# rapidsai/cugraph

Measured on NVIDIA H100. Metric: MTEPS (million traversed edges/sec) PageRank RMAT-24 ef-16, 100 iterations, higher is better.
Workload: dtype f32

## Files before the change

cugraph_b200/csrc/graph.cuh:

```cuda
#pragma once
#include "common.cuh"

#include <memory>
#include <vector>

namespace b200 {

constexpr int kNumSeg                = 7;
constexpr int kSegThreshold[kNumSeg] = {32, 16, 8, 4, 2, 1, 0};

constexpr int kWarpChunk  = 1024;
constexpr int kWarpsPerCta = 8;

struct sweep_cache_t;

struct csx_t {
  int32_t n_rows{0};
  int64_t nnz{0};
  bool offs64{false};
  dbuf offsets;
  dbuf indices;
  dbuf weights;
  dbuf row_vertex;
  bool degree_sorted{true};
  int32_t seg[kNumSeg + 1]{};
  int64_t nnz_hi{0};
  int32_t n_chunks{0};
  dbuf chunk_first_row;
  int32_t n_split{0};
  dbuf split_rows;
  mutable std::unique_ptr<sweep_cache_t> sweep;
  mutable dbuf out_w;
  csx_t();
  ~csx_t();
};

struct graph_impl {
  cugraph_data_type_id_t vertex_type{INT32};
  cugraph_data_type_id_t edge_type{INT32};
  cugraph_data_type_id_t weight_type{FLOAT32};
  bool weighted{false};
  bool is_symmetric{false};
  bool is_multigraph{false};
  bool store_transposed{false};
  bool renumbered{true};
  int32_t n_vertices{0};
  int64_t n_edges{0};
  int device{0};

  dbuf ext_of_int;
  dbuf sorted_ext;
  dbuf int_of_rank;

  std::unique_ptr<csx_t> primary;
  std::unique_ptr<csx_t> pull_alt;
  std::unique_ptr<csx_t> push_alt;
  std::unique_ptr<csx_t> out_alt;
};

inline graph_impl* G(cugraph_graph_t* g)
{
  B200_EXPECTS(g != nullptr, CUGRAPH_INVALID_INPUT, "graph is NULL");
  return reinterpret_cast<graph_impl*>(g);
}

csx_t const& pull_view(handle_impl const& h, graph_impl& g);
csx_t const& push_view(handle_impl const& h, graph_impl& g);
csx_t const& out_sweep_view(handle_impl const& h, graph_impl& g);

struct pr_state_t {
  double diff;
  double dangling;
  double init;
  double pers_scale;
  double last_diff;
  int iter;
  int done;
};
struct sweep_scratch_t {
  dbuf acc, state;
  void init(handle_impl const& h, csx_t const& c);
  void set_init(handle_impl const& h, double init);
  pr_state_t* st() const { return state.as<pr_state_t>(); }
};
size_t padded_x_elems(int32_t n_vertices, size_t elem_size);
template <typename T>
dbuf make_sweep_x(handle_impl const& h, int32_t n_vertices);
template <typename T>
void pull_sweep(handle_impl const& h, csx_t const& c, int32_t n_vertices, T const* x, T* y, sweep_scratch_t& sc, double alpha,
                bool use_weights = true, bool covered_rows_only = false);
void prepare_pull_sweep(handle_impl const& h, csx_t const& c, int32_t n_vertices, size_t elem_size);

void ext_to_int(handle_impl const& h, graph_impl const& g, void const* ext, size_t n, int32_t* out);
void int_to_ext(handle_impl const& h, graph_impl const& g, int32_t const* in, size_t n, void* ext_out);
dbuf reported_vertices(handle_impl const& h, graph_impl const& g);
dbuf to_reported_order(handle_impl const& h, graph_impl const& g, void const* internal_vals, size_t elem_size);

template <typename T>
dbuf collect_vertex_values(handle_impl const& h, graph_impl const& g,
                           device_array_view_impl const* verts, device_array_view_impl const* vals,
                           T fill);

std::unique_ptr<csx_t> build_binned_rows(handle_impl const& h, int32_t const* major, int32_t const* minor, void const* w,
                                         cugraph_data_type_id_t wtype, int64_t n, int32_t nv);
dbuf expand_majors(handle_impl const& h, csx_t const& c);

}
```

cugraph_b200/csrc/pagerank.cu:

```cuda
#include "graph.cuh"

#include <algorithm>
#include <cmath>

namespace b200 {
namespace {

__global__ void k_out_degree(int32_t const* __restrict__ indices, long long nnz, int32_t* __restrict__ deg)
{
  for (long long i = blockIdx.x * (long long)blockDim.x + threadIdx.x; i < nnz; i += (long long)gridDim.x * blockDim.x)
    atomicAdd(deg + indices[i], 1);
}

template <typename T>
__global__ void k_out_weight(int32_t const* __restrict__ indices, T const* __restrict__ w, long long nnz, double* __restrict__ sums)
{
  for (long long i = blockIdx.x * (long long)blockDim.x + threadIdx.x; i < nnz; i += (long long)gridDim.x * blockDim.x)
    atomicAdd(sums + indices[i], (double)w[i]);
}

template <typename S, typename T>
__global__ void k_cast(S const* in, int32_t n, T* out)
{
  for (int64_t i = blockIdx.x * (int64_t)blockDim.x + threadIdx.x; i < n; i += (int64_t)gridDim.x * blockDim.x) out[i] = (T)in[i];
// ... 1 lines not shown

template <typename T>
__global__ void __launch_bounds__(kBlock)
k_vertex_pass(T const* __restrict__ pr_new, T const* __restrict__ pr_old, T const* __restrict__ out_w,
              T* __restrict__ x, int32_t n, pr_state_t* __restrict__ st)
{
  if (st->done) return;
  __shared__ double smem[8];
  double diff = 0.0, dang = 0.0;
  for (int i = blockIdx.x * blockDim.x + threadIdx.x; i < n; i += gridDim.x * blockDim.x) {
    T nv = pr_new[i];
    T ow = out_w[i];
    if (pr_old) diff += fabs((double)nv - (double)pr_old[i]);
    if (ow == (T)0) dang += (double)nv;
    x[i] = (ow == (T)0) ? nv : nv / ow;
  }
  diff = block_sum(diff, smem);
  dang = block_sum(dang, smem);
  if (threadIdx.x == 0) {
    if (pr_old) atomicAdd(&st->diff, diff);
    atomicAdd(&st->dangling, dang);
  }
}

__global__ void k_finalize(pr_state_t* st, double alpha, double epsilon, int n_vertices, int personalized,
                           int count_iteration, int max_iterations)
{
  if (st->done) return;
  double base    = st->dangling * alpha + (1.0 - alpha);
  st->init       = personalized ? 0.0 : base / (double)n_vertices;
  st->pers_scale = base;
  if (count_iteration) {
    st->iter += 1;
    st->last_diff = st->diff;
    if (st->diff < epsilon || st->iter >= max_iterations) st->done = 1;
  }
  st->diff     = 0.0;
  st->dangling = 0.0;
}

template <typename T>
__global__ void k_personalize(int32_t const* __restrict__ pv, T const* __restrict__ pvals, int32_t n, double pers_sum,
                              T* __restrict__ y, pr_state_t const* __restrict__ st)
{
  if (st->done) return;
  for (int64_t i = blockIdx.x * (int64_t)blockDim.x + threadIdx.x; i < n; i += (int64_t)gridDim.x * blockDim.x)
    y[pv[i]] = (T)((double)y[pv[i]] + st->pers_scale * ((double)pvals[i] / pers_sum));
}

template <typename T>
__global__ void k_sum(T const* a, int32_t n, double* out)
{
  __shared__ double smem[8];
  double s = 0.0;
  for (int i = blockIdx.x * blockDim.x + threadIdx.x; i < n; i += gridDim.x * blockDim.x) s += (double)a[i];
  s = block_sum(s, smem);
  if (threadIdx.x == 0) atomicAdd(out, s);
}

struct pr_args {
  device_array_view_impl const* pre_v{nullptr};
  device_array_view_impl const* pre_w{nullptr};
  device_array_view_impl const* init_v{nullptr};
  device_array_view_impl const* init_val{nullptr};
  device_array_view_impl const* pers_v{nullptr};
  device_array_view_impl const* pers_val{nullptr};
  double alpha{0.85};
  double epsilon{1e-5};
  size_t max_iterations{100};
  bool expensive{false};
};

template <typename T>
void pagerank_typed(handle_impl const& h, graph_impl& g, pr_args const& a, centrality_result_impl& res)
{
  phase_trace tr(h);
  const int32_t nv = g.n_vertices;
  B200_EXPECTS(a.alpha >= 0.0 && a.alpha <= 1.0, CUGRAPH_UNKNOWN_ERROR, "Invalid input argument: alpha should be in [0.0, 1.0].");
  B200_EXPECTS(a.epsilon >= 0.0, CUGRAPH_UNKNOWN_ERROR, "Invalid input argument: epsilon should be non-negative.");
  if (nv == 0) {
    res.vertices   = new device_array_impl{dbuf(0, h.stream), 0, g.vertex_type};
    res.values     = new device_array_impl{dbuf(0, h.stream), 0, g.weight_type};
    res.iterations = 0;
    res.converged  = true;
    return;
  }
  csx_t const& c = pull_view(h, g);
  B200_EXPECTS(c.degree_sorted, CUGRAPH_UNKNOWN_ERROR, "internal: pull view is not binned");
  const bool weighted = g.weighted;

  dbuf out_w_user;
  T const* out_w = nullptr;
  if (a.pre_w) {
    out_w_user = collect_vertex_values<T>(h, g, a.pre_v, a.pre_w, (T)0);
    out_w      = out_w_user.as<T>();
  } else {
    if (c.out_w.data() == nullptr) {
      dbuf ow = make_dbuf<T>(nv, h.stream);
      if (weighted) {
        dbuf sums = make_dbuf<double>(nv, h.stream);
        CUDA_TRY(cudaMemsetAsync(sums.data(), 0, sizeof(double) * nv, h.stream));
        if (c.nnz > 0)
          B200_LAUNCH(h, (k_out_weight<T>), grid_for(c.nnz, 1, h.sm_count * 16), kBlock, 0, c.indices.as<int32_t>(),
                      c.weights.as<T>(), (long long)c.nnz, sums.as<double>());
        B200_LAUNCH(h, (k_cast<double, T>), grid_for(nv), kBlock, 0, sums.as<double>(), nv, ow.as<T>());
      } else {
        dbuf deg = make_dbuf<int32_t>(nv, h.stream);
        CUDA_TRY(cudaMemsetAsync(deg.data(), 0, sizeof(int32_t) * nv, h.stream));
        if (c.nnz > 0)
          B200_LAUNCH(h, k_out_degree, grid_for(c.nnz, 1, h.sm_count * 16), kBlock, 0, c.indices.as<int32_t>(),
                      (long long)c.nnz, deg.as<int32_t>());
        B200_LAUNCH(h, (k_cast<int32_t, T>), grid_for(nv), kBlock, 0, deg.as<int32_t>(), nv, ow.as<T>());
      }
      sync(h);
      c.out_w = std::move(ow);
    }
    out_w = c.out_w.as<T>();
  }
  tr.mark("pagerank: pull view + out-weights");
  if (a.expensive && weighted && c.nnz > 0) {
    dbuf neg = make_dbuf<int>(1, h.stream);
    CUDA_TRY(cudaMemsetAsync(neg.data(), 0, sizeof(int), h.stream));
    B200_LAUNCH(h, (k_count_negative<T>), grid_for(c.nnz, 1, h.sm_count * 16), kBlock, 0, c.weights.as<T>(), c.nnz, neg.as<int>());
    B200_EXPECTS(read_back(h, neg.as<int>()) == 0, CUGRAPH_UNKNOWN_ERROR, "Invalid input argument: input edge weights should have non-negative values.");
  }

  dbuf pers_idx, pers_vals;
  int32_t n_pers  = 0;
  double pers_sum = 0.0;
  if (a.pers_v) {
    B200_EXPECTS(a.pers_val && a.pers_v->size == a.pers_val->size, CUGRAPH_UNKNOWN_ERROR,
                 "Invalid input argument: if personalization.has_value() is true, the size of vertices and values should match");
    B200_EXPECTS(a.pers_v->size > 0, CUGRAPH_UNKNOWN_ERROR,
                 "Invalid input argument: if personalizations.has_value() is true, the input personalization vector size should not be 0.");
    n_pers   = (int32_t)a.pers_v->size;
    pers_idx = make_dbuf<int32_t>(n_pers, h.stream);
    ext_to_int(h, g, a.pers_v->data, n_pers, pers_idx.as<int32_t>());
    struct pers_check_t {
      double sum;
      int n_invalid;
    };
    dbuf chk = make_dbuf<pers_check_t>(1, h.stream);
    auto* dchk = chk.as<pers_check_t>();
    CUDA_TRY(cudaMemsetAsync(dchk, 0, sizeof(pers_check_t), h.stream));
    B200_LAUNCH(h, (k_count_negative<int32_t>), grid_for(n_pers), kBlock, 0, pers_idx.as<int32_t>(), (int64_t)n_pers, &dchk->n_invalid);
    B200_LAUNCH(h, (k_sum<T>), grid_for(n_pers, 1, 1024), kBlock, 0, (T const*)a.pers_val->data, n_pers, &dchk->sum);
    const pers_check_t hchk = read_back(h, dchk);
    B200_EXPECTS(hchk.n_invalid == 0, CUGRAPH_INVALID_INPUT, "Invalid input argument: peresonalization vertices have invalid vertex IDs.");
    pers_sum = hchk.sum;
    B200_EXPECTS(pers_sum > 0.0, CUGRAPH_UNKNOWN_ERROR, "Invalid input argument: sum of personalization valuese should be positive.");
  }

  dbuf pr_a = make_dbuf<T>(nv, h.stream), pr_b = make_dbuf<T>(nv, h.stream);
  dbuf x    = make_sweep_x<T>(h, nv);
  sweep_scratch_t sc;
  sc.init(h, c);
  pr_state_t* st = sc.st();

  if (a.init_val) {
    dbuf guess = collect_vertex_values<T>(h, g, a.init_v, a.init_val, (T)0);
    CUDA_TRY(cudaMemcpyAsync(pr_a.data(), guess.data(), sizeof(T) * nv, cudaMemcpyDeviceToDevice, h.stream));
    sync(h);
  } else {
    B200_LAUNCH(h, (k_fill<T>), grid_for(nv), kBlock, 0, pr_a.as<T>(), nv, (T)((T)1 / (T)nv));
  }

  tr.mark("pagerank: state setup");
  const int vgrid = grid_for(nv, 1, h.sm_count * 8);
  const int max_it = (int)std::min<size_t>(a.max_iterations, 0x7fffffff);
  B200_LAUNCH(h, (k_vertex_pass<T>), vgrid, kBlock, 0, pr_a.as<T>(), (T const*)nullptr, out_w, x.as<T>(), nv, st);
  B200_LAUNCH(h, k_finalize, 1, 1, 0, st, a.alpha, a.epsilon, nv, n_pers > 0 ? 1 : 0, 0, max_it);

  T* cur = pr_a.as<T>();
  T* nxt = pr_b.as<T>();
  pr_state_t* hst = reinterpret_cast<pr_state_t*>(h.pinned);
  int enqueued    = 0;
  int iters       = 0;
  const int batch = (a.epsilon > 0.0) ? 8 : 64;
  while (true) {
    int todo = std::min(batch, std::max(max_it, 1) - enqueued);
    for (int k = 0; k < todo; ++k) {
      pull_sweep<T>(h, c, nv, x.as<T>(), nxt, sc, a.alpha);
      if (n_pers > 0)
        B200_LAUNCH(h, (k_personalize<T>), grid_for(n_pers), kBlock, 0, pers_idx.as<int32_t>(), (T const*)a.pers_val->data,
                    n_pers, pers_sum, nxt, st);
      B200_LAUNCH(h, (k_vertex_pass<T>), vgrid, kBlock, 0, nxt, cur, out_w, x.as<T>(), nv, st);
      B200_LAUNCH(h, k_finalize, 1, 1, 0, st, a.alpha, a.epsilon, nv, n_pers > 0 ? 1 : 0, 1, max_it);
      std::swap(cur, nxt);
      ++enqueued;
    }
    check_last("pagerank iteration");
    CUDA_TRY(cudaMemcpyAsync(hst, st, sizeof(pr_state_t), cudaMemcpyDeviceToHost, h.stream));
    sync(h);
    iters = hst->iter;
    if (hst->done || enqueued >= std::max(max_it, 1)) break;
  }
  tr.mark("pagerank: iterations (+ layout staging on the first call)");
  T* final_pr = (iters % 2 == 0) ? pr_a.as<T>() : pr_b.as<T>();

  res.vertices   = new device_array_impl{reported_vertices(h, g), (size_t)nv, g.vertex_type};
  res.values     = new device_array_impl{to_reported_order(h, g, final_pr, sizeof(T)), (size_t)nv, g.weight_type};
  res.iterations = (size_t)iters;
  res.converged  = (size_t)iters < a.max_iterations;
  sync(h);
  tr.mark("pagerank: result gather");
}

cugraph_error_code_t pagerank_entry(const cugraph_resource_handle_t* handle, cugraph_graph_t* graph, pr_args a,
                                    bool require_convergence, cugraph_centrality_result_t** result,
                                    cugraph_error_t** error)
{
  return guarded(error, [&] {
    auto const& h = H(handle);
    auto* g       = G(graph);
    B200_EXPECTS(result != nullptr, CUGRAPH_INVALID_INPUT, "result out-pointer is NULL");
    *result = nullptr;
    if (a.pre_v) {
      B200_EXPECTS(a.pre_v->type == g->vertex_type, CUGRAPH_INVALID_INPUT,
                   "vertex type of graph and precomputed_vertex_out_weight_vertices must match");
      B200_EXPECTS(a.pre_w && a.pre_w->type == g->weight_type, CUGRAPH_INVALID_INPUT,
                   "vertex type of graph and precomputed_vertex_out_weight_sums must match");
    }
    if (a.init_v) {
      B200_EXPECTS(a.init_v->type == g->vertex_type, CUGRAPH_INVALID_INPUT,
                   "vertex type of graph and initial_guess_vertices must match");
      B200_EXPECTS(a.init_val && a.init_val->type == g->weight_type, CUGRAPH_INVALID_INPUT,
                   "vertex type of graph and initial_guess_values must match");
    }
    if (a.pers_v) {
      B200_EXPECTS(a.pers_v->type == g->vertex_type, CUGRAPH_INVALID_INPUT,
                   "vertex type of graph and personalization_vector must match");
      B200_EXPECTS(a.pers_val && a.pers_val->type == g->weight_type, CUGRAPH_INVALID_INPUT,
                   "vertex type of graph and personalization_vector must match");
    }
    if (!a.pre_w) a.pre_v = nullptr;
    if (!a.init_val) a.init_v = nullptr;
    auto res = std::make_unique<centrality_result_impl>();
    if (g->weight_type == FLOAT32) pagerank_typed<float>(h, *g, a, *res);
    else pagerank_typed<double>(h, *g, a, *res);
    bool converged = res->converged;
    *result        = reinterpret_cast<cugraph_centrality_result_t*>(res.release());
    B200_EXPECTS(!require_convergence || converged, CUGRAPH_UNKNOWN_ERROR, "PageRank failed to converge.");
  });
}

}

}

using namespace b200;

extern "C" {

cugraph_type_erased_device_array_view_t* cugraph_centrality_result_get_vertices(cugraph_centrality_result_t* result)
{
  auto* r = reinterpret_cast<centrality_result_impl*>(result);
  return reinterpret_cast<cugraph_type_erased_device_array_view_t*>(r->vertices->new_view());
}

cugraph_type_erased_device_array_view_t* cugraph_centrality_result_get_values(cugraph_centrality_result_t* result)
{
  auto* r = reinterpret_cast<centrality_result_impl*>(result);
  return reinterpret_cast<cugraph_type_erased_device_array_view_t*>(r->values->new_view());
}

size_t cugraph_centrality_result_get_num_iterations(cugraph_centrality_result_t* result)
{
  return reinterpret_cast<centrality_result_impl*>(result)->iterations;
}

bool_t cugraph_centrality_result_converged(cugraph_centrality_result_t* result)
{
  return reinterpret_cast<centrality_result_impl*>(result)->converged ? TRUE : FALSE;
}

void cugraph_centrality_result_free(cugraph_centrality_result_t* result)
{
  if (!result) return;
  auto* r = reinterpret_cast<centrality_result_impl*>(result);
  delete r->vertices;
  delete r->values;
  delete r;
}

#define PR_ARGS_COMMON                                                                          \
  pr_args a;                                                                                    \
  a.pre_v          = V(precomputed_vertex_out_weight_vertices);                                 \
  a.pre_w          = V(precomputed_vertex_out_weight_sums);                                     \
  a.init_v         = V(initial_guess_vertices);                                                 \
  a.init_val       = V(initial_guess_values);                                                   \
  a.alpha          = alpha;                                                                     \
  a.epsilon        = epsilon;                                                                   \
  a.max_iterations = max_iterations;                                                            \
  a.expensive      = do_expensive_check == TRUE;

cugraph_error_code_t cugraph_pagerank(const cugraph_resource_handle_t* handle, cugraph_graph_t* graph,
                                      const cugraph_type_erased_device_array_view_t* precomputed_vertex_out_weight_vertices,
                                      const cugraph_type_erased_device_array_view_t* precomputed_vertex_out_weight_sums,
                                      const cugraph_type_erased_device_array_view_t* initial_guess_vertices,
                                      const cugraph_type_erased_device_array_view_t* initial_guess_values, double alpha,
                                      double epsilon, size_t max_iterations, bool_t do_expensive_check,
                                      cugraph_centrality_result_t** result, cugraph_error_t** error)
{
  PR_ARGS_COMMON
  return pagerank_entry(handle, graph, a, true, result, error);
}

cugraph_error_code_t cugraph_pagerank_allow_nonconvergence(
  const cugraph_resource_handle_t* handle, cugraph_graph_t* graph,
  const cugraph_type_erased_device_array_view_t* precomputed_vertex_out_weight_vertices,
  const cugraph_type_erased_device_array_view_t* precomputed_vertex_out_weight_sums,
  const cugraph_type_erased_device_array_view_t* initial_guess_vertices,
  const cugraph_type_erased_device_array_view_t* initial_guess_values, double alpha, double epsilon,
  size_t max_iterations, bool_t do_expensive_check, cugraph_centrality_result_t** result, cugraph_error_t** error)
{
  PR_ARGS_COMMON
  return pagerank_entry(handle, graph, a, false, result, error);
}

cugraph_error_code_t cugraph_personalized_pagerank(
  const cugraph_resource_handle_t* handle, cugraph_graph_t* graph,
  const cugraph_type_erased_device_array_view_t* precomputed_vertex_out_weight_vertices,
  const cugraph_type_erased_device_array_view_t* precomputed_vertex_out_weight_sums,
  const cugraph_type_erased_device_array_view_t* initial_guess_vertices,
  const cugraph_type_erased_device_array_view_t* initial_guess_values,
  const cugraph_type_erased_device_array_view_t* personalization_vertices,
  const cugraph_type_erased_device_array_view_t* personalization_values, double alpha, double epsilon,
  size_t max_iterations, bool_t do_expensive_check, cugraph_centrality_result_t** result, cugraph_error_t** error)
{
  PR_ARGS_COMMON
  a.pers_v   = V(personalization_vertices);
  a.pers_val = V(personalization_values);
  return pagerank_entry(handle, graph, a, true, result, error);
}

cugraph_error_code_t cugraph_personalized_pagerank_allow_nonconvergence(
  const cugraph_resource_handle_t* handle, cugraph_graph_t* graph,
  const cugraph_type_erased_device_array_view_t* precomputed_vertex_out_weight_vertices,
  const cugraph_type_erased_device_array_view_t* precomputed_vertex_out_weight_sums,
  const cugraph_type_erased_device_array_view_t* initial_guess_vertices,
  const cugraph_type_erased_device_array_view_t* initial_guess_values,
// ... 47 lines not shown
```

cugraph_b200/csrc/sweep.cu:

```cuda
#include "sweep.cuh"

namespace b200 {
namespace {

inline int32_t acc_rows(csx_t const& c) { return std::max(c.n_rows, 1); }

template <typename T>
__global__ void k_fill_pattern(T* x, int32_t n)
{
  for (int64_t i = blockIdx.x * (int64_t)blockDim.x + threadIdx.x; i < n; i += (int64_t)gridDim.x * blockDim.x)
    x[i] = (T)(0.5 + (double)(((unsigned)i * 2654435761u) >> 16) / 65536.0);
}

template <typename T>
__global__ void k_compare_rows(int32_t const* __restrict__ row_vertex, T const* __restrict__ a, T const* __restrict__ b,
                               int32_t n_rows, int32_t n_hi, double tol, unsigned long long* __restrict__ worst ,
                               unsigned long long* __restrict__ n_bad )
{
  for (int64_t r = blockIdx.x * (int64_t)blockDim.x + threadIdx.x; r < n_rows; r += (int64_t)gridDim.x * blockDim.x) {
    const int v     = row_vertex ? row_vertex[r] : (int)r;
    const double va = (double)a[v], vb = (double)b[v];
    const double den = fmax(fabs(va), 1e-300);
    const float rel  = (float)fmin(fabs(va - vb) / den, 1e30);
    const int cls    = r < n_hi ? 0 : 1;
    atomicMax(worst + cls, ((unsigned long long)__float_as_uint(rel) << 32) | (unsigned)r);
    if (rel > tol) atomicAdd(n_bad + cls, 1ull);
  }
}

}

void sweep_scratch_t::init(handle_impl const& h, csx_t const& c)
{
  acc = make_dbuf<double>(acc_rows(c), h.stream);
  CUDA_TRY(cudaMemsetAsync(acc.data(), 0, sizeof(double) * acc_rows(c), h.stream));
  state = make_dbuf<pr_state_t>(1, h.stream);
  CUDA_TRY(cudaMemsetAsync(state.data(), 0, sizeof(pr_state_t), h.stream));
}

void sweep_scratch_t::set_init(handle_impl const& h, double init)
{
  pr_state_t hs{};
  hs.init = init;
  CUDA_TRY(cudaMemcpyAsync(state.data(), &hs, sizeof(pr_state_t), cudaMemcpyHostToDevice, h.stream));
  sync(h);
}

size_t padded_x_elems(int32_t n_vertices, size_t elem_size)
{
  const size_t slice = kHotSliceBytes / elem_size;
  const size_t W     = slice - kHotZeroPad;
  return ((size_t)n_vertices / W + 2) * slice;
}

template <typename T>
dbuf make_sweep_x(handle_impl const& h, int32_t n_vertices)
{
  const size_t n = padded_x_elems(n_vertices, sizeof(T));
  dbuf x         = make_dbuf<T>(n, h.stream);
  CUDA_TRY(cudaMemsetAsync(x.data(), 0, n * sizeof(T), h.stream));
  return x;
}

template <typename T>
void pull_sweep(handle_impl const& h, csx_t const& c, int32_t n_vertices, T const* x, T* y, sweep_scratch_t& sc, double alpha,
                bool use_weights, bool covered_rows_only)
{
  double* acc = sc.acc.as<double>();
  if (sweep_layout_t const* L = sweep_layout(h, c, n_vertices, sizeof(T)))
    launch_sweep<T>(h, c, *L, x, y, acc, alpha, sc.st(), use_weights, covered_rows_only);
  else if (c.offs64)
    launch_pull_sweep<int64_t, T>(h, c, x, y, acc, alpha, sc.st(), use_weights);
  else
    launch_pull_sweep<int32_t, T>(h, c, x, y, acc, alpha, sc.st(), use_weights);
}

void prepare_pull_sweep(handle_impl const& h, csx_t const& c, int32_t nv, size_t es) { sweep_layout(h, c, nv, es); }

template dbuf make_sweep_x<float>(handle_impl const&, int32_t);
template dbuf make_sweep_x<double>(handle_impl const&, int32_t);
template void pull_sweep(handle_impl const&, csx_t const&, int32_t, float const*, float*, sweep_scratch_t&, double, bool, bool);
template void pull_sweep(handle_impl const&, csx_t const&, int32_t, double const*, double*, sweep_scratch_t&, double, bool, bool);

}

using namespace b200;

extern "C" {

cugraph_error_code_t cugraph_b200_debug_compare_sweeps(const cugraph_resource_handle_t* handle, cugraph_graph_t* graph,
                                                       double* out, cugraph_error_t** error)
{
  return guarded(error, [&] {
    auto const& h = H(handle);
    auto* g       = G(graph);
    B200_EXPECTS(out != nullptr, CUGRAPH_INVALID_INPUT, "out is NULL");
    B200_EXPECTS(g->weight_type == FLOAT32, CUGRAPH_NOT_IMPLEMENTED, "single-GPU float32 graphs only");
    csx_t const& c = pull_view(h, *g);
    B200_EXPECTS(!c.offs64, CUGRAPH_NOT_IMPLEMENTED, "32-bit offsets only");
    const int32_t nv = g->n_vertices;
    dbuf x = make_sweep_x<float>(h, nv), y0 = make_dbuf<float>(nv, h.stream), y1 = make_dbuf<float>(nv, h.stream);
    B200_LAUNCH(h, (k_fill_pattern<float>), grid_for(nv), kBlock, 0, x.as<float>(), nv);
    sweep_scratch_t sc;
    sc.init(h, c);
    launch_pull_sweep<int32_t, float>(h, c, x.as<float>(), y0.as<float>(), sc.acc.as<double>(), 0.85, sc.st());
    pull_sweep<float>(h, c, nv, x.as<float>(), y1.as<float>(), sc, 0.85);
    dbuf res = make_dbuf<unsigned long long>(4, h.stream);
    CUDA_TRY(cudaMemsetAsync(res.data(), 0, 4 * sizeof(unsigned long long), h.stream));
    B200_LAUNCH(h, (k_compare_rows<float>), grid_for(c.n_rows), kBlock, 0, c.row_vertex.as<int32_t>(), y0.as<float>(), y1.as<float>(), c.n_rows, c.seg[0], 1e-5,
                res.as<unsigned long long>(), res.as<unsigned long long>() + 2);
    unsigned long long hres[4];
    CUDA_TRY(cudaMemcpyAsync(hres, res.data(), sizeof(hres), cudaMemcpyDeviceToHost, h.stream));
    sync(h);
    for (int k = 0; k < 2; ++k) {
      const unsigned bits = (unsigned)(hres[k] >> 32);
      float rel;
      std::memcpy(&rel, &bits, sizeof(rel));
      const int32_t row = (int32_t)(hres[k] & 0xffffffffu);
      int32_t offs[2]   = {0, 0};
      if (c.n_rows > 0)
        CUDA_TRY(cudaMemcpy(offs, c.offsets.as<int32_t>() + row, sizeof(offs), cudaMemcpyDeviceToHost));
      out[4 * k + 0] = rel;
      out[4 * k + 1] = row;
      out[4 * k + 2] = offs[1] - offs[0];
      out[4 * k + 3] = (double)hres[2 + k];
    }
    check_last("debug_compare_sweeps");
  });
}

}
```

cugraph_b200/csrc/sweep.cuh:

```cuda
#pragma once
#include "spmv.cuh"
#include "sweep_layout.cuh"

namespace b200 {

constexpr int kSweepThreads = 512;
constexpr int kSweepWarps   = kSweepThreads / 32;
constexpr int kSweepDynSmem = kHotSliceBytes;
constexpr int kTmaPiece     = 16 * 1024;
constexpr int kStealMin     = 12;

#ifndef B200_HOST_EMU
__device__ __forceinline__ uint32_t smem_u32(const void* p) { return (uint32_t)__cvta_generic_to_shared(p); }

__device__ __forceinline__ void mbar_init(uint64_t* bar, unsigned count)
{
  asm volatile("mbarrier.init.shared::cta.b64 [%0], %1;" ::"r"(smem_u32(bar)), "r"(count));
  asm volatile("fence.mbarrier_init.release.cluster;" ::: "memory");
}
__device__ __forceinline__ void mbar_expect_tx(uint64_t* bar, unsigned bytes)
{
  asm volatile("mbarrier.arrive.expect_tx.shared::cta.b64 _, [%0], %1;" ::"r"(smem_u32(bar)), "r"(bytes) : "memory");
}
__device__ __forceinline__ void mbar_wait(uint64_t* bar, unsigned parity)
// ... 357 lines not shown
__device__ __forceinline__ int draw_get(int raw) { return __shfl_sync(0xffffffffu, raw, 0); }

__device__ __forceinline__ uint4 batch_headers(sweep_chunk_t const* __restrict__ chunks, int first, int cnt, int lane)
{
  uint4 v = make_uint4(0u, 0u, 0u, 0xffffffffu);
  if (lane < cnt) v = ld_stream_v4(chunks + first + lane);
  return v;
}

struct chunk_supply_t {
  sweep_chunk_t const* __restrict__ chunks;
  int* cursor;
  uint4* ring;
  int n;
  uint4 pend;
  int cnt_cur, cnt_nxt, j, slot;
  int raw_nn, want_nn;

  __device__ __forceinline__ void start(sweep_chunk_t const* __restrict__ c, int* cur, uint4* warp_ring, int n_chunks, int lane)
  {
    chunks = c;
    cursor = cur;
    ring   = warp_ring;
    n      = n_chunks;
    const int w0 = draw_want(n, 0);
    const int r0 = draw_issue(cursor, w0, lane, true), r1 = draw_issue(cursor, w0, lane, true);
    const int b0 = draw_get(r0);
    cnt_cur      = b0 < n ? (n - b0 < w0 ? n - b0 : w0) : 0;
    const uint4 v0 = batch_headers(chunks, b0, cnt_cur, lane);
    const int b1 = draw_get(r1);
    cnt_nxt      = b1 < n ? (n - b1 < w0 ? n - b1 : w0) : 0;
    pend         = batch_headers(chunks, b1, cnt_nxt, lane);
    want_nn      = draw_want(n, b1 < n ? b1 + w0 : n);
    raw_nn       = draw_issue(cursor, want_nn, lane, b1 + w0 < n);
    j            = 0;
    slot         = 0;
    __syncwarp();
    if (lane < kDrawMax) ring[lane] = v0;
    __syncwarp();
  }
  __device__ __forceinline__ sweep_chunk_t next(int lane)
  {
    if (j == cnt_cur && cnt_cur > 0) {
      slot ^= 1;
      if (lane < kDrawMax) ring[slot * kDrawMax + lane] = pend;
      __syncwarp();
      cnt_cur = cnt_nxt;
      j       = 0;
      const int b2 = draw_get(raw_nn);
      cnt_nxt      = b2 < n ? (n - b2 < want_nn ? n - b2 : want_nn) : 0;
      pend         = batch_headers(chunks, b2, cnt_nxt, lane);
      const int w3 = draw_want(n, b2 < n ? b2 + want_nn : n);
      raw_nn       = draw_issue(cursor, w3, lane, b2 + want_nn < n);
      want_nn      = w3;
    }
    sweep_chunk_t ch;
    ch.kind = -1;
    ch.n_groups = ch.sr_begin = ch.row_begin = 0;
    if (cnt_cur > 0) {
      const uint4 h = ring[slot * kDrawMax + j];
      ++j;
      ch.sr_begin  = (int)h.x;
      ch.row_begin = (int)h.y;
      ch.n_groups  = (int)h.z;
      ch.kind      = (int)h.w;
    }
    return ch;
  }
};

template <typename T, bool WEIGHTED>
__global__ void __launch_bounds__(kSweepThreads, 1) k_sweep(sweep_args_t<T> a)
{
  B200_DYN_SMEM(smem_raw);
  T* sx = reinterpret_cast<T*>(smem_raw);
  __shared__ uint64_t bar;
  __shared__ int s_best;
  __shared__ uint4 s_ring[kSweepWarps][2 * kDrawMax];
  if (a.st->done) return;
  a.p.pol        = make_l2_policy_evict_first();
  a.p.acc_pol    = make_l2_policy_evict_last();
  const int lane = threadIdx.x & 31;
  const int me   = (int)blockIdx.x;
  if (threadIdx.x == 0) mbar_init(&bar, 1);
  if (threadIdx.x < kHotZeroPad) sx[a.W + threadIdx.x] = (T)0;
  const int own_lo = a.cta_phase[me], own_hi = a.cta_phase[me + 1];
  int next_own    = own_lo;
  unsigned parity = 0;
  int cur_block   = -1;
  while (true) {
    int p = -1;
    if (next_own < own_hi) {
      p = next_own++;
    } else {
      if (threadIdx.x == 0) s_best = 0;
      __syncthreads();
      int best = 0;
      for (int q = a.ph_lo + (int)threadIdx.x; q < a.ph_hi; q += kSweepThreads) {
        if (q >= own_lo && q < own_hi) continue;
        const sweep_phase_t ph = a.phases[q];
        const int left         = (ph.chunk_end - ph.chunk_begin) - ld_volatile(a.cursor + q);
        if (left >= kStealMin && left > best) best = left;
      }
      if (best > 0) atomicMax(&s_best, best);
      __syncthreads();
      const int win = s_best;
      __syncthreads();
      if (win > 0) {
        if (threadIdx.x == 0) s_best = a.ph_hi;
        __syncthreads();
        for (int q = a.ph_lo + (int)threadIdx.x; q < a.ph_hi; q += kSweepThreads) {
          if (q >= own_lo && q < own_hi) continue;
          const sweep_phase_t ph = a.phases[q];
          const int left         = (ph.chunk_end - ph.chunk_begin) - ld_volatile(a.cursor + q);
          if (left >= kStealMin && left * 2 >= win) atomicMin(&s_best, q);
        }
        __syncthreads();
        p = s_best < a.ph_hi ? s_best : -1;
      }
    }
    __syncthreads();
    if (p < 0) break;
    const sweep_phase_t ph = a.phases[p];
    const int n            = ph.chunk_end - ph.chunk_begin;
    const bool fresh       = ph.block != cur_block;
    if (fresh) {
      if (threadIdx.x == 0) load_slice(smem_raw, a.x, ph.block, a.W, &bar);
      cur_block = ph.block;
    }
    chunk_supply_t sup;
    sup.start(a.chunks + ph.chunk_begin, a.cursor + p, s_ring[threadIdx.x >> 5], n, lane);
    sweep_chunk_t hA = sup.next(lane);
    sweep_chunk_t hB = sup.next(lane);
    chunk_regs_t A, B;
    chunk_load(A, hA, a.p, lane);
    if (fresh) {
      mbar_wait(&bar, parity);
      parity ^= 1;
    }
    while (hA.kind >= 0) {
      chunk_load(B, hB, a.p, lane);
      const sweep_chunk_t hC = sup.next(lane);
      chunk_process<T, WEIGHTED>(A, hA, a.p, sx, lane);
      if (hB.kind < 0) break;
      chunk_load(A, hC, a.p, lane);
      const sweep_chunk_t hD = sup.next(lane);
      chunk_process<T, WEIGHTED>(B, hB, a.p, sx, lane);
      hA = hC;
      hB = hD;
    }
  }
}

template <typename T, int kFinishSteps>
__global__ void __launch_bounds__(256)
k_sweep_finish(double* __restrict__ acc, int row_lo, int n_cov, int n_rows, T* __restrict__ y, int32_t const* __restrict__ row_vertex,
               double alpha, int* __restrict__ cursor, int n_phases, pr_state_t const* __restrict__ st)
{
  static_assert(kBandRowAlign % (64 * kFinishSteps) == 0, "a warp's rows must not straddle a band bound");
  if (st->done) return;
  const int t = blockIdx.x * blockDim.x + threadIdx.x;
  if (t < n_phases) cursor[t] = 0;
  const int lane = threadIdx.x & 31;
  const int base = row_lo + (t >> 5) * (64 * kFinishSteps) + 2 * lane;
  if (base - 2 * lane >= n_rows) return;
  const double init = st->init;
  double2 q[kFinishSteps];
#pragma unroll
  for (int k = 0; k < kFinishSteps; ++k) {
    const int r = base + 64 * k;
    q[k]        = make_double2(0.0, 0.0);
    if (r + 1 < n_cov) q[k] = *reinterpret_cast<double2*>(acc + r);
    else if (r < n_cov) q[k].x = acc[r];
  }
#pragma unroll
  for (int k = 0; k < kFinishSteps; ++k) {
    const int r = base + 64 * k;
    if (r + 1 < n_cov) *reinterpret_cast<double2*>(acc + r) = make_double2(0.0, 0.0);
    else if (r < n_cov) acc[r] = 0.0;
    const T v0 = (T)(q[k].x * alpha + init), v1 = (T)(q[k].y * alpha + init);
    if (!row_vertex && r + 1 < n_rows && sizeof(T) == 4) {
      *reinterpret_cast<float2*>(y + r) = make_float2((float)v0, (float)v1);
    } else {
      if (r < n_rows) y[row_vertex ? row_vertex[r] : r] = v0;
      if (r + 1 < n_rows) y[row_vertex ? row_vertex[r + 1] : r + 1] = v1;
    }
  }
}

constexpr int kTailThreads = 512;
constexpr int kTailBatch   = 8;

#ifndef B200_HOST_EMU
__device__ __forceinline__ float ld_keep(float const* p, unsigned long long pol)
{
  float v;
  asm("ld.global.nc.L2::cache_hint.f32 %0, [%1], %2;" : "=f"(v) : "l"(p), "l"(pol));
  return v;
}
__device__ __forceinline__ double ld_keep(double const* p, unsigned long long pol)
{
  double v;
  asm("ld.global.nc.L2::cache_hint.f64 %0, [%1], %2;" : "=d"(v) : "l"(p), "l"(pol));
  return v;
}
#else
inline float ld_keep(float const* p, unsigned long long) { return *p; }
inline double ld_keep(double const* p, unsigned long long) { return *p; }
#endif

template <typename T>
struct tail_args_t {
  tail_run_t const* __restrict__ runs;
  int32_t const* __restrict__ ids;
  T const* __restrict__ w;
  T const* __restrict__ x;
  T* __restrict__ y;
  int32_t const* __restrict__ row_vertex;
  int* __restrict__ cursor;
  pr_state_t const* __restrict__ st;
  int n_runs, empty_hi, W;
  double alpha;
};

struct tail_unit_t {
  int d, n_tiles, row0, row_end;
  long long base;
};

__device__ __forceinline__ tail_unit_t tail_unit(tail_run_t const* runs, int n_runs, int u)
{
  tail_unit_t t{0, 0, 0, 0, 0};
  if (u >= runs[n_runs].first_unit) return t;
  int r = 0;
  while (u >= runs[r + 1].first_unit) ++r;
  const tail_run_t R = runs[r];
  const int per      = tail_unit_tiles(R.degree);
  const int tile     = (u - R.first_unit) * per;
  t.d                = R.degree;
  const int left     = runs[r + 1].first_tile - R.first_tile - tile;
  t.n_tiles          = left < per ? left : per;
  t.row0             = R.first_row + tile * kTailTile;
  t.row_end          = runs[r + 1].first_row;
  t.base             = R.id_off + (long long)tile * kTailTile * R.degree;
  return t;
}

__device__ __forceinline__ void tail_load(int (&q)[kTailUnitEntries], tail_unit_t const& u, int32_t const* __restrict__ ids,
                                          unsigned long long pol, int lane)
{
  const int n         = u.n_tiles * u.d;
  int32_t const* base = ids + u.base + lane;
#pragma unroll
  for (int j = 0; j < kTailUnitEntries; ++j)
    if (j < n) q[j] = ld_stream_i32(base + j * kTailTile, pol);
}

template <typename T, bool WEIGHTED, int D>
__device__ __forceinline__ void tail_rows(int const (&q)[kTailUnitEntries], tail_unit_t const& u, tail_args_t<T> const& a,
                                          T const* __restrict__ sx, double init, unsigned long long pol, unsigned long long keep,
                                          int lane)
{
  constexpr int U = tail_unit_tiles(D);
  T const* wp       = WEIGHTED ? a.w + u.base + lane : nullptr;
#pragma unroll
  for (int t = 0; t < U; ++t) {
    if (t < u.n_tiles) {
      double s = 0.0;
#pragma unroll
      for (int k0 = 0; k0 < D; k0 += kTailBatch) {
        double b[kTailBatch];
#pragma unroll
        for (int i = 0; i < kTailBatch; ++i) {
          b[i] = 0.0;
          if (k0 + i < D) {
            const int j = t * D + k0 + i;
            const int c = j < kTailUnitEntries ? q[j] : ld_stream_i32(a.ids + u.base + j * kTailTile + lane, pol);
            T v         = c < a.W ? sx[c] : ld_keep(a.x + c, keep);
            if (WEIGHTED) v *= ld_stream(wp + j * kTailTile);
            b[i] = (double)v;
          }
        }
        s += ((b[0] + b[1]) + (b[2] + b[3])) + ((b[4] + b[5]) + (b[6] + b[7]));
      }
      const int row = u.row0 + t * kTailTile + lane;
      if (row < u.row_end) a.y[a.row_vertex ? a.row_vertex[row] : row] = (T)(s * a.alpha + init);
    }
  }
}

template <typename T, bool WEIGHTED, int D = 1>
__device__ __forceinline__ void tail_process(int const (&q)[kTailUnitEntries], tail_unit_t const& u, tail_args_t<T> const& a,
                                             T const* __restrict__ sx, double init, unsigned long long pol,
                                             unsigned long long keep, int lane)
{
  if (u.d == D) tail_rows<T, WEIGHTED, D>(q, u, a, sx, init, pol, keep, lane);
  else if constexpr (D < kTailMaxDegree) tail_process<T, WEIGHTED, D + 1>(q, u, a, sx, init, pol, keep, lane);
}

template <typename T, bool WEIGHTED>
__global__ void __launch_bounds__(kTailThreads, 1) k_sweep_tail(tail_args_t<T> a)
{
  B200_DYN_SMEM(smem_raw);
  T const* sx = reinterpret_cast<T const*>(smem_raw);
  __shared__ uint64_t bar;
  __shared__ tail_run_t s_run[kTailMaxDegree + 1];
  if (a.st->done) return;
  const unsigned long long pol = make_l2_policy_evict_first(), keep = make_l2_policy_evict_last();
  const int lane = threadIdx.x & 31;
  if (threadIdx.x == 0) {
    mbar_init(&bar, 1);
    load_slice(smem_raw, a.x, 0, a.W, &bar);
  }
  if ((int)threadIdx.x <= a.n_runs) s_run[threadIdx.x] = a.runs[threadIdx.x];
  const double init = a.st->init;
  __syncthreads();
  const int ra = draw_issue(a.cursor, 1, lane, true), rb = draw_issue(a.cursor, 1, lane, true);
  tail_unit_t A = tail_unit(s_run, a.n_runs, draw_get(ra));
  int qa[kTailUnitEntries], qb[kTailUnitEntries];
  tail_load(qa, A, a.ids, pol, lane);
  tail_unit_t B = tail_unit(s_run, a.n_runs, draw_get(rb));
  mbar_wait(&bar, 0);
  while (A.d > 0) {
    tail_load(qb, B, a.ids, pol, lane);
    const int rc = draw_issue(a.cursor, 1, lane, B.d > 0);
    tail_process<T, WEIGHTED>(qa, A, a, sx, init, pol, keep, lane);
    if (B.d == 0) break;
    const tail_unit_t C = tail_unit(s_run, a.n_runs, draw_get(rc));
    tail_load(qa, C, a.ids, pol, lane);
    const int rd = draw_issue(a.cursor, 1, lane, C.d > 0);
    tail_process<T, WEIGHTED>(qb, B, a, sx, init, pol, keep, lane);
    A = C;
    B = tail_unit(s_run, a.n_runs, draw_get(rd));
  }
  const int stride = gridDim.x * blockDim.x;
  for (int r = a.runs[a.n_runs].first_row + (int)(blockIdx.x * blockDim.x + threadIdx.x); r < a.empty_hi; r += stride)
    a.y[a.row_vertex ? a.row_vertex[r] : r] = (T)init;
}

template <typename T>
void launch_sweep(handle_impl const& h, csx_t const& c, sweep_layout_t const& L, T const* x, T* y, double* acc, double alpha,
                  pr_state_t const* st, bool use_weights, bool covered_rows_only)
{
  const bool weighted = use_weights && L.w.data() != nullptr;
  auto* const sweep_kernel = weighted ? k_sweep<T, true> : k_sweep<T, false>;
  auto* const tail_kernel  = weighted ? k_sweep_tail<T, true> : k_sweep_tail<T, false>;
  CUDA_TRY(cudaFuncSetAttribute(sweep_kernel, cudaFuncAttributeMaxDynamicSharedMemorySize, kSweepDynSmem));
  sweep_args_t<T> a;
  a.p.ids     = L.ids.as<uint4>();
  a.p.rows    = L.rows.as<int32_t>();
  a.p.w       = L.w.data();
  a.p.acc     = acc;
  a.chunks    = L.chunks.as<sweep_chunk_t>();
  a.phases    = L.phases.as<sweep_phase_t>();
  a.cursor    = L.cursor.as<int>();
  a.x         = x;
  a.st        = st;
  a.W         = L.W;
  a.p.pol     = 0;
  a.p.acc_pol = 0;
  constexpr int kFinishSteps = 8;
  const int32_t finish_rows = covered_rows_only ? L.n_cov : c.n_rows;
  const bool tail           = L.n_str < L.n_cov;
  for (int band = 0; band < L.n_bands; ++band) {
    const int row_hi = band < L.n_bands - 1 ? L.band_row[band + 1] : (tail ? L.n_str : finish_rows);
    const int row_lo = L.band_row[band];
    a.cta_phase      = L.cta_phase.as<int32_t>() + (size_t)band * L.n_cta;
    a.ph_lo          = L.band_phase[band];
    a.ph_hi          = L.band_phase[band + 1];
    B200_LAUNCH(h, sweep_kernel, L.n_cta, kSweepThreads, kSweepDynSmem, a);
    const int n_ph = a.ph_hi - a.ph_lo + (band == L.n_bands - 1 && tail ? 1 : 0);
    const int n    = std::max((row_hi - row_lo + 2 * kFinishSteps - 1) / (2 * kFinishSteps), n_ph);
    B200_LAUNCH(h, (k_sweep_finish<T, kFinishSteps>), (std::max(n, 1) + 255) / 256, 256, 0, acc, row_lo, L.n_str, row_hi, y,
                c.row_vertex.as<int32_t>(), alpha, L.cursor.as<int>() + a.ph_lo, n_ph, st);
  }
  if (tail) {
    tail_args_t<T> t;
    t.runs       = L.tail_run.as<tail_run_t>();
    t.ids        = L.tail_ids.as<int32_t>();
    t.w          = weighted ? L.tail_w.as<T>() : nullptr;
    t.x          = x;
    t.y          = y;
    t.row_vertex = c.row_vertex.as<int32_t>();
    t.cursor     = L.cursor.as<int>() + L.n_phases;
    t.st         = st;
    t.n_runs     = L.n_tail_runs;
    t.empty_hi   = finish_rows;
    t.W          = L.W;
    t.alpha      = alpha;
    const int units  = L.tail_runs.back().first_unit;
    const int blocks = std::max(1, std::min(h.sm_count, (units + kTailThreads / 32 - 1) / (kTailThreads / 32)));
    CUDA_TRY(cudaFuncSetAttribute(tail_kernel, cudaFuncAttributeMaxDynamicSharedMemorySize, kSweepDynSmem));
    B200_LAUNCH(h, tail_kernel, blocks, kTailThreads, kSweepDynSmem, t);
  }
}

}
```

Measured before the change: 386,600.

## Fuse PageRank vertex pass into sweep finish and tail kernels

Moves the per-vertex PageRank update (diff, dangling sum, scaled x for the next iteration) into the epilogues of the sweep finish and tail kernels, and double-buffers x so the next-iteration vector can be written while the current one is still being read. This drops the separate k_vertex_pass launch and its extra full pass over pr_new, pr_old and out_w each iteration when there is no personalization. The cost is more register pressure and a block reduction with atomics in the finish and tail kernels, plus a second x buffer.

```diff
diff --git a/cugraph_b200/csrc/graph.cuh b/cugraph_b200/csrc/graph.cuh
--- a/cugraph_b200/csrc/graph.cuh
+++ b/cugraph_b200/csrc/graph.cuh
@@ -89,6 +89,9 @@
 template <typename T>
 void pull_sweep(handle_impl const& h, csx_t const& c, int32_t n_vertices, T const* x, T* y, sweep_scratch_t& sc, double alpha,
                 bool use_weights = true, bool covered_rows_only = false);
+template <typename T>
+bool pagerank_pull_sweep(handle_impl const& h, csx_t const& c, int32_t n_vertices, T const* x, T* pr_new, T const* pr_old,
+                         T const* out_w, T* x_next, sweep_scratch_t& sc, double alpha);
 void prepare_pull_sweep(handle_impl const& h, csx_t const& c, int32_t n_vertices, size_t elem_size);
 
 void ext_to_int(handle_impl const& h, graph_impl const& g, void const* ext, size_t n, int32_t* out);
diff --git a/cugraph_b200/csrc/pagerank.cu b/cugraph_b200/csrc/pagerank.cu
--- a/cugraph_b200/csrc/pagerank.cu
+++ b/cugraph_b200/csrc/pagerank.cu
@@ -177,7 +177,7 @@
   }
 
   dbuf pr_a = make_dbuf<T>(nv, h.stream), pr_b = make_dbuf<T>(nv, h.stream);
-  dbuf x    = make_sweep_x<T>(h, nv);
+  dbuf x_a = make_sweep_x<T>(h, nv), x_b = make_sweep_x<T>(h, nv);
   sweep_scratch_t sc;
   sc.init(h, c);
   pr_state_t* st = sc.st();
@@ -193,11 +193,13 @@
   tr.mark("pagerank: state setup");
   const int vgrid = grid_for(nv, 1, h.sm_count * 8);
   const int max_it = (int)std::min<size_t>(a.max_iterations, 0x7fffffff);
-  B200_LAUNCH(h, (k_vertex_pass<T>), vgrid, kBlock, 0, pr_a.as<T>(), (T const*)nullptr, out_w, x.as<T>(), nv, st);
+  B200_LAUNCH(h, (k_vertex_pass<T>), vgrid, kBlock, 0, pr_a.as<T>(), (T const*)nullptr, out_w, x_a.as<T>(), nv, st);
   B200_LAUNCH(h, k_finalize, 1, 1, 0, st, a.alpha, a.epsilon, nv, n_pers > 0 ? 1 : 0, 0, max_it);
 
   T* cur = pr_a.as<T>();
   T* nxt = pr_b.as<T>();
+  T* x_cur = x_a.as<T>();
+  T* x_nxt = x_b.as<T>();
   pr_state_t* hst = reinterpret_cast<pr_state_t*>(h.pinned);
   int enqueued    = 0;
   int iters       = 0;
@@ -205,13 +207,18 @@
   while (true) {
     int todo = std::min(batch, std::max(max_it, 1) - enqueued);
     for (int k = 0; k < todo; ++k) {
-      pull_sweep<T>(h, c, nv, x.as<T>(), nxt, sc, a.alpha);
-      if (n_pers > 0)
+      bool passed = false;
+      if (n_pers > 0) {
+        pull_sweep<T>(h, c, nv, x_cur, nxt, sc, a.alpha);
         B200_LAUNCH(h, (k_personalize<T>), grid_for(n_pers), kBlock, 0, pers_idx.as<int32_t>(), (T const*)a.pers_val->data,
                     n_pers, pers_sum, nxt, st);
-      B200_LAUNCH(h, (k_vertex_pass<T>), vgrid, kBlock, 0, nxt, cur, out_w, x.as<T>(), nv, st);
+      } else {
+        passed = pagerank_pull_sweep<T>(h, c, nv, x_cur, nxt, cur, out_w, x_nxt, sc, a.alpha);
+      }
+      if (!passed) B200_LAUNCH(h, (k_vertex_pass<T>), vgrid, kBlock, 0, nxt, cur, out_w, x_nxt, nv, st);
       B200_LAUNCH(h, k_finalize, 1, 1, 0, st, a.alpha, a.epsilon, nv, n_pers > 0 ? 1 : 0, 1, max_it);
       std::swap(cur, nxt);
+      std::swap(x_cur, x_nxt);
       ++enqueued;
     }
     check_last("pagerank iteration");
diff --git a/cugraph_b200/csrc/sweep.cu b/cugraph_b200/csrc/sweep.cu
--- a/cugraph_b200/csrc/sweep.cu
+++ b/cugraph_b200/csrc/sweep.cu
@@ -75,12 +75,30 @@
     launch_pull_sweep<int32_t, T>(h, c, x, y, acc, alpha, sc.st(), use_weights);
 }
 
+template <typename T>
+bool pagerank_pull_sweep(handle_impl const& h, csx_t const& c, int32_t n_vertices, T const* x, T* pr_new, T const* pr_old,
+                         T const* out_w, T* x_next, sweep_scratch_t& sc, double alpha)
+{
+  sweep_layout_t const* L = sweep_layout(h, c, n_vertices, sizeof(T));
+  if (!L) {
+    pull_sweep<T>(h, c, n_vertices, x, pr_new, sc, alpha);
+    return false;
+  }
+  const pr_epilogue_t<T> pr{pr_old, out_w, x_next, sc.st()};
+  launch_sweep<T>(h, c, *L, x, pr_new, sc.acc.as<double>(), alpha, sc.st(), true, false, &pr);
+  return true;
+}
+
 void prepare_pull_sweep(handle_impl const& h, csx_t const& c, int32_t nv, size_t es) { sweep_layout(h, c, nv, es); }
 
 template dbuf make_sweep_x<float>(handle_impl const&, int32_t);
 template dbuf make_sweep_x<double>(handle_impl const&, int32_t);
 template void pull_sweep(handle_impl const&, csx_t const&, int32_t, float const*, float*, sweep_scratch_t&, double, bool, bool);
 template void pull_sweep(handle_impl const&, csx_t const&, int32_t, double const*, double*, sweep_scratch_t&, double, bool, bool);
+template bool pagerank_pull_sweep(handle_impl const&, csx_t const&, int32_t, float const*, float*, float const*, float const*,
+                                  float*, sweep_scratch_t&, double);
+template bool pagerank_pull_sweep(handle_impl const&, csx_t const&, int32_t, double const*, double*, double const*,
+                                  double const*, double*, sweep_scratch_t&, double);
 
 }
 
diff --git a/cugraph_b200/csrc/sweep.cuh b/cugraph_b200/csrc/sweep.cuh
--- a/cugraph_b200/csrc/sweep.cuh
+++ b/cugraph_b200/csrc/sweep.cuh
@@ -533,10 +533,58 @@
   }
 }
 
-template <typename T, int kFinishSteps>
+template <typename T>
+struct pr_epilogue_t {
+  T const* __restrict__ pr_old;
+  T const* __restrict__ out_w;
+  T* __restrict__ x_next;
+  pr_state_t* __restrict__ st;
+};
+
+template <typename T> struct vec2_of;
+template <> struct vec2_of<float> { using type = float2; };
+template <> struct vec2_of<double> { using type = double2; };
+
+template <typename T>
+__device__ __forceinline__ T pr_vertex(T val, T old, T ow, double& diff, double& dang)
+{
+  diff += fabs((double)val - (double)old);
+  if (ow == (T)0) dang += (double)val;
+  return ow == (T)0 ? val : val / ow;
+}
+template <typename T>
+__device__ __forceinline__ void pr_row(pr_epilogue_t<T> const& e, T* __restrict__ pr_new, int v, T val, double& diff, double& dang)
+{
+  pr_new[v]   = val;
+  e.x_next[v] = pr_vertex(val, e.pr_old[v], e.out_w[v], diff, dang);
+}
+template <typename T>
+__device__ __forceinline__ void pr_row_pair(pr_epilogue_t<T> const& e, T* __restrict__ pr_new, int v, T v0, T v1, double& diff,
+                                            double& dang)
+{
+  using V2      = typename vec2_of<T>::type;
+  const V2 old  = *reinterpret_cast<V2 const*>(e.pr_old + v);
+  const V2 ow   = *reinterpret_cast<V2 const*>(e.out_w + v);
+  *reinterpret_cast<V2*>(pr_new + v) = V2{v0, v1};
+  const T x0 = pr_vertex(v0, old.x, ow.x, diff, dang), x1 = pr_vertex(v1, old.y, ow.y, diff, dang);
+  *reinterpret_cast<V2*>(e.x_next + v) = V2{x0, x1};
+}
+template <typename T>
+__device__ __forceinline__ void pr_flush(pr_epilogue_t<T> const& e, double diff, double dang)
+{
+  __shared__ double smem[32];
+  diff = block_sum(diff, smem);
+  dang = block_sum(dang, smem);
+  if (threadIdx.x == 0) {
+    atomicAdd(&e.st->diff, diff);
+    atomicAdd(&e.st->dangling, dang);
+  }
+}
+
+template <typename T, int kFinishSteps, bool PR>
 __global__ void __launch_bounds__(256)
 k_sweep_finish(double* __restrict__ acc, int row_lo, int n_cov, int n_rows, T* __restrict__ y, int32_t const* __restrict__ row_vertex,
-               double alpha, int* __restrict__ cursor, int n_phases, pr_state_t const* __restrict__ st)
+               double alpha, int* __restrict__ cursor, int n_phases, pr_state_t const* __restrict__ st, pr_epilogue_t<T> pr)
 {
   static_assert(kBandRowAlign % (64 * kFinishSteps) == 0, "a warp's rows must not straddle a band bound");
   if (st->done) return;
@@ -544,29 +592,39 @@
   if (t < n_phases) cursor[t] = 0;
   const int lane = threadIdx.x & 31;
   const int base = row_lo + (t >> 5) * (64 * kFinishSteps) + 2 * lane;
-  if (base - 2 * lane >= n_rows) return;
+  const bool live = base - 2 * lane < n_rows;
+  if (!PR && !live) return;
   const double init = st->init;
+  double diff = 0.0, dang = 0.0;
   double2 q[kFinishSteps];
 #pragma unroll
   for (int k = 0; k < kFinishSteps; ++k) {
     const int r = base + 64 * k;
     q[k]        = make_double2(0.0, 0.0);
-    if (r + 1 < n_cov) q[k] = *reinterpret_cast<double2*>(acc + r);
-    else if (r < n_cov) q[k].x = acc[r];
+    if (live && r + 1 < n_cov) q[k] = *reinterpret_cast<double2*>(acc + r);
+    else if (live && r < n_cov) q[k].x = acc[r];
   }
 #pragma unroll
   for (int k = 0; k < kFinishSteps; ++k) {
     const int r = base + 64 * k;
-    if (r + 1 < n_cov) *reinterpret_cast<double2*>(acc + r) = make_double2(0.0, 0.0);
-    else if (r < n_cov) acc[r] = 0.0;
+    if (live && r + 1 < n_cov) *reinterpret_cast<double2*>(acc + r) = make_double2(0.0, 0.0);
+    else if (live && r < n_cov) acc[r] = 0.0;
     const T v0 = (T)(q[k].x * alpha + init), v1 = (T)(q[k].y * alpha + init);
-    if (!row_vertex && r + 1 < n_rows && sizeof(T) == 4) {
+    if constexpr (PR) {
+      if (!row_vertex && r + 1 < n_rows) {
+        pr_row_pair(pr, y, r, v0, v1, diff, dang);
+      } else {
+        if (r < n_rows) pr_row(pr, y, row_vertex ? row_vertex[r] : r, v0, diff, dang);
+        if (r + 1 < n_rows) pr_row(pr, y, row_vertex ? row_vertex[r + 1] : r + 1, v1, diff, dang);
+      }
+    } else if (!row_vertex && r + 1 < n_rows && sizeof(T) == 4) {
       *reinterpret_cast<float2*>(y + r) = make_float2((float)v0, (float)v1);
     } else {
       if (r < n_rows) y[row_vertex ? row_vertex[r] : r] = v0;
       if (r + 1 < n_rows) y[row_vertex ? row_vertex[r + 1] : r + 1] = v1;
     }
   }
+  if constexpr (PR) pr_flush(pr, diff, dang);
 }
 
 constexpr int kTailThreads = 512;
@@ -602,6 +660,7 @@
   pr_state_t const* __restrict__ st;
   int n_runs, empty_hi, W;
   double alpha;
+  pr_epilogue_t<T> pr;
 };
 
 struct tail_unit_t {
@@ -637,16 +696,26 @@
     if (j < n) q[j] = ld_stream_i32(base + j * kTailTile, pol);
 }
 
-template <typename T, bool WEIGHTED, int D>
+template <typename T, bool WEIGHTED, bool PR, int D>
 __device__ __forceinline__ void tail_rows(int const (&q)[kTailUnitEntries], tail_unit_t const& u, tail_args_t<T> const& a,
                                           T const* __restrict__ sx, double init, unsigned long long pol, unsigned long long keep,
-                                          int lane)
+                                          int lane, double& diff, double& dang)
 {
   constexpr int U = tail_unit_tiles(D);
   T const* wp       = WEIGHTED ? a.w + u.base + lane : nullptr;
 #pragma unroll
   for (int t = 0; t < U; ++t) {
     if (t < u.n_tiles) {
+      const int row = u.row0 + t * kTailTile + lane;
+      int v  = 0;
+      T old  = (T)0, ow = (T)0;
+      if constexpr (PR) {
+        if (row < u.row_end) {
+          v   = a.row_vertex ? a.row_vertex[row] : row;
+          old = a.pr.pr_old[v];
+          ow  = a.pr.out_w[v];
+        }
+      }
       double s = 0.0;
 #pragma unroll
       for (int k0 = 0; k0 < D; k0 += kTailBatch) {
@@ -664,22 +733,29 @@
         }
         s += ((b[0] + b[1]) + (b[2] + b[3])) + ((b[4] + b[5]) + (b[6] + b[7]));
       }
-      const int row = u.row0 + t * kTailTile + lane;
-      if (row < u.row_end) a.y[a.row_vertex ? a.row_vertex[row] : row] = (T)(s * a.alpha + init);
-    }
-  }
-}
-
-template <typename T, bool WEIGHTED, int D = 1>
+      if (row < u.row_end) {
+        if constexpr (PR) {
+          const T val    = (T)(s * a.alpha + init);
+          a.y[v]         = val;
+          a.pr.x_next[v] = pr_vertex(val, old, ow, diff, dang);
+        } else {
+          a.y[a.row_vertex ? a.row_vertex[row] : row] = (T)(s * a.alpha + init);
+        }
+      }
+    }
+  }
+}
+
+template <typename T, bool WEIGHTED, bool PR, int D = 1>
 __device__ __forceinline__ void tail_process(int const (&q)[kTailUnitEntries], tail_unit_t const& u, tail_args_t<T> const& a,
                                              T const* __restrict__ sx, double init, unsigned long long pol,
-                                             unsigned long long keep, int lane)
-{
-  if (u.d == D) tail_rows<T, WEIGHTED, D>(q, u, a, sx, init, pol, keep, lane);
-  else if constexpr (D < kTailMaxDegree) tail_process<T, WEIGHTED, D + 1>(q, u, a, sx, init, pol, keep, lane);
-}
-
-template <typename T, bool WEIGHTED>
+                                             unsigned long long keep, int lane, double& diff, double& dang)
+{
+  if (u.d == D) tail_rows<T, WEIGHTED, PR, D>(q, u, a, sx, init, pol, keep, lane, diff, dang);
+  else if constexpr (D < kTailMaxDegree) tail_process<T, WEIGHTED, PR, D + 1>(q, u, a, sx, init, pol, keep, lane, diff, dang);
+}
+
+template <typename T, bool WEIGHTED, bool PR>
 __global__ void __launch_bounds__(kTailThreads, 1) k_sweep_tail(tail_args_t<T> a)
 {
   B200_DYN_SMEM(smem_raw);
@@ -695,6 +771,7 @@
   }
   if ((int)threadIdx.x <= a.n_runs) s_run[threadIdx.x] = a.runs[threadIdx.x];
   const double init = a.st->init;
+  double diff = 0.0, dang = 0.0;
   __syncthreads();
   const int ra = draw_issue(a.cursor, 1, lane, true), rb = draw_issue(a.cursor, 1, lane, true);
   tail_unit_t A = tail_unit(s_run, a.n_runs, draw_get(ra));
@@ -705,27 +782,58 @@
   while (A.d > 0) {
     tail_load(qb, B, a.ids, pol, lane);
     const int rc = draw_issue(a.cursor, 1, lane, B.d > 0);
-    tail_process<T, WEIGHTED>(qa, A, a, sx, init, pol, keep, lane);
+    tail_process<T, WEIGHTED, PR>(qa, A, a, sx, init, pol, keep, lane, diff, dang);
     if (B.d == 0) break;
     const tail_unit_t C = tail_unit(s_run, a.n_runs, draw_get(rc));
     tail_load(qa, C, a.ids, pol, lane);
     const int rd = draw_issue(a.cursor, 1, lane, C.d > 0);
-    tail_process<T, WEIGHTED>(qb, B, a, sx, init, pol, keep, lane);
+    tail_process<T, WEIGHTED, PR>(qb, B, a, sx, init, pol, keep, lane, diff, dang);
     A = C;
     B = tail_unit(s_run, a.n_runs, draw_get(rd));
   }
   const int stride = gridDim.x * blockDim.x;
-  for (int r = a.runs[a.n_runs].first_row + (int)(blockIdx.x * blockDim.x + threadIdx.x); r < a.empty_hi; r += stride)
-    a.y[a.row_vertex ? a.row_vertex[r] : r] = (T)init;
+  const int first  = a.runs[a.n_runs].first_row + (int)(blockIdx.x * blockDim.x + threadIdx.x);
+  if constexpr (PR) {
+    constexpr int kEmptyBatch = 4;
+    for (int r0 = first; r0 < a.empty_hi; r0 += kEmptyBatch * stride) {
+      int v[kEmptyBatch];
+      T old[kEmptyBatch], ow[kEmptyBatch];
+#pragma unroll
+      for (int i = 0; i < kEmptyBatch; ++i) {
+        const int r = r0 + i * stride;
+        v[i]        = r < a.empty_hi ? (a.row_vertex ? a.row_vertex[r] : r) : -1;
+      }
+#pragma unroll
+      for (int i = 0; i < kEmptyBatch; ++i) {
+        old[i] = ow[i] = (T)0;
+        if (v[i] >= 0) {
+          old[i] = a.pr.pr_old[v[i]];
+          ow[i]  = a.pr.out_w[v[i]];
+        }
+      }
+#pragma unroll
+      for (int i = 0; i < kEmptyBatch; ++i) {
+        if (v[i] >= 0) {
+          a.y[v[i]]         = (T)init;
+          a.pr.x_next[v[i]] = pr_vertex((T)init, old[i], ow[i], diff, dang);
+        }
+      }
+    }
+    pr_flush(a.pr, diff, dang);
+  } else {
+    for (int r = first; r < a.empty_hi; r += stride) a.y[a.row_vertex ? a.row_vertex[r] : r] = (T)init;
+  }
 }
 
 template <typename T>
 void launch_sweep(handle_impl const& h, csx_t const& c, sweep_layout_t const& L, T const* x, T* y, double* acc, double alpha,
-                  pr_state_t const* st, bool use_weights, bool covered_rows_only)
+                  pr_state_t const* st, bool use_weights, bool covered_rows_only, pr_epilogue_t<T> const* pr = nullptr)
 {
   const bool weighted = use_weights && L.w.data() != nullptr;
   auto* const sweep_kernel = weighted ? k_sweep<T, true> : k_sweep<T, false>;
-  auto* const tail_kernel  = weighted ? k_sweep_tail<T, true> : k_sweep_tail<T, false>;
+  auto* const tail_kernel  = pr ? (weighted ? k_sweep_tail<T, true, true> : k_sweep_tail<T, false, true>)
+                                : (weighted ? k_sweep_tail<T, true, false> : k_sweep_tail<T, false, false>);
+  const pr_epilogue_t<T> epi = pr ? *pr : pr_epilogue_t<T>{};
   CUDA_TRY(cudaFuncSetAttribute(sweep_kernel, cudaFuncAttributeMaxDynamicSharedMemorySize, kSweepDynSmem));
   sweep_args_t<T> a;
   a.p.ids     = L.ids.as<uint4>();
@@ -741,6 +849,7 @@
   a.p.pol     = 0;
   a.p.acc_pol = 0;
   constexpr int kFinishSteps = 8;
+  auto* const finish_kernel = pr ? k_sweep_finish<T, kFinishSteps, true> : k_sweep_finish<T, kFinishSteps, false>;
   const int32_t finish_rows = covered_rows_only ? L.n_cov : c.n_rows;
   const bool tail           = L.n_str < L.n_cov;
   for (int band = 0; band < L.n_bands; ++band) {
@@ -752,8 +861,8 @@
     B200_LAUNCH(h, sweep_kernel, L.n_cta, kSweepThreads, kSweepDynSmem, a);
     const int n_ph = a.ph_hi - a.ph_lo + (band == L.n_bands - 1 && tail ? 1 : 0);
     const int n    = std::max((row_hi - row_lo + 2 * kFinishSteps - 1) / (2 * kFinishSteps), n_ph);
-    B200_LAUNCH(h, (k_sweep_finish<T, kFinishSteps>), (std::max(n, 1) + 255) / 256, 256, 0, acc, row_lo, L.n_str, row_hi, y,
-                c.row_vertex.as<int32_t>(), alpha, L.cursor.as<int>() + a.ph_lo, n_ph, st);
+    B200_LAUNCH(h, finish_kernel, (std::max(n, 1) + 255) / 256, 256, 0, acc, row_lo, L.n_str, row_hi, y,
+                c.row_vertex.as<int32_t>(), alpha, L.cursor.as<int>() + a.ph_lo, n_ph, st, epi);
   }
   if (tail) {
     tail_args_t<T> t;
@@ -769,6 +878,7 @@
     t.empty_hi   = finish_rows;
     t.W          = L.W;
     t.alpha      = alpha;
+    t.pr         = epi;
     const int units  = L.tail_runs.back().first_unit;
     const int blocks = std::max(1, std::min(h.sm_count, (units + kTailThreads / 32 - 1) / (kTailThreads / 32)));
     CUDA_TRY(cudaFuncSetAttribute(tail_kernel, cudaFuncAttributeMaxDynamicSharedMemorySize, kSweepDynSmem));
```

Result: faster. 391,700 (median of 6 runs) (+1.3%).
